# valeoai/NAF

Measured on AMD Instinct MI355X. Metric: upsampled Mpixels/sec (NAF forward), higher is better.
Workload: dtype bf16; 1 GPU; G1: 1x3x1024x1024 guidance, 1x768x64x64 features -> 1024x1024, window 7, per GPU; per_gpu_batch=1, global_batch=1, parallelism=batch-shard x1, scope=whole forward (conv stem + RoPE/pool + attention), weights=random-init NAF() defaults (dim 256, 4 heads), streams=2

## Files before the change

### naf_amd/csrc/stem_conv1x1.hip

```cpp
#include <type_traits>

#include "naf_common.h"

struct StemConv1Params {
    const bf16_t* x;
    bf16_t* y;
    const bf16_t* w;
    const float* bias;
    const float* gamma;
    const float* beta;
    const double* stats_in;
    double* stats_out;
    int32_t B, H, W;
    int32_t groups_per_image;
    int32_t groups_per_block;
    float eps;
    int64_t xs[3], ys[3];
    const void* img;
    const float* w0;
    const float* b0;
    int64_t ibs;
    int32_t is[4];
    bf16_t* kout;
    const float* tab_y;
    const float* tab_x;
    int64_t kst[3];
    int32_t cw;
    int32_t ncell;
    int32_t cells_per_block;
};

namespace {
constexpr int C1 = 128, WROW = C1 + 8, OROW1 = C1 + 8;
#ifndef NAF_C1X1_NW
#define NAF_C1X1_NW 4
#endif
#ifndef NAF_C1_ABL
#define NAF_C1_ABL 0
#endif
constexpr int NW1 = NAF_C1X1_NW;
typedef float f32x16_t __attribute__((ext_vector_type(16)));
constexpr float kLog2e = 1.4426950408889634f;
}

#ifdef NAF_C1_TIMING
__device__ unsigned long long g_c1_tim[4096 * 8];
#define C1_T(i) do { const unsigned long long now_ = __builtin_amdgcn_s_memtime(); tacc[i] += now_ - tlast; tlast = now_; } while (0)
#else
#define C1_T(i) do { } while (0)
#endif

template <bool IMG, typename T, bool DENSE, bool PLAIN = false, bool POOL = false>
__global__ __launch_bounds__(NW1 * 64, (NW1 <= 4 ? 2 : 1)) void stem_conv1x1_kernel(const StemConv1Params p) {
    static_assert(!(IMG && PLAIN), "the recomputed-conv0 input exists for the forward layer only");
    static_assert(!POOL || (DENSE && !IMG && !PLAIN), "key pooling: dense forward layer reading its input from memory");
#ifdef NAF_C1_TIMING
    unsigned long long tacc[8] = {0, 0, 0, 0, 0, 0, 0, 0}, tlast = __builtin_amdgcn_s_memtime();
#endif
    extern __shared__ __attribute__((aligned(16))) unsigned char smem[];
    bf16_t* wl = reinterpret_cast<bf16_t*>(smem);
    bf16_t* ot = wl + C1 * WROW;
    float* cvec = reinterpret_cast<float*>(ot + NW1 * 32 * OROW1);

    const int tid = threadIdx.x, lane = tid & 63;
    const int wave = __builtin_amdgcn_readfirstlane(tid >> 6);
    const int n32 = lane & 31, half = lane >> 5;
    const int b = blockIdx.y;

    const int gbase = POOL ? blockIdx.x * p.cells_per_block : blockIdx.x * p.groups_per_block;
    const int ngroups = POOL ? min(p.ncell, gbase + p.cells_per_block) : min(p.groups_per_image, gbase + p.groups_per_block);
    const int gstride = NW1;
    const int npx = p.H * p.W;
    bf16_t* otw = ot + wave * 32 * OROW1;

    const int chk = lane & 15, psub = lane >> 4;
    const bool xdense = DENSE || p.xs[1] == (int64_t)p.W * p.xs[2], ydense = DENSE || p.ys[1] == (int64_t)p.W * p.ys[2];
    const bf16_t* xbase = p.x + b * p.xs[0] + chk * 8;
    const uint32_t lane_x = (uint32_t)(psub * (int)p.xs[2] + chk * 8) * 2u, lane_y = (uint32_t)(psub * (int)p.ys[2] + chk * 8) * 2u;
    const int nfull = npx >> 5;
    auto pool_group_off = [&](int cell, int gi, const int64_t (&st)[3]) __attribute__((always_inline)) {
        const int cc = cell < ngroups ? cell : ngroups - 1;
        const int cy = cc / p.cw, cx = cc - cy * p.cw;
        return (int64_t)(cy * 16 + 2 * gi) * st[1] + (int64_t)cx * 16 * st[2];
    };
    auto load_group = [&](int g, u32x4_t (&raw)[8], int gi = 0) __attribute__((always_inline)) {
        if constexpr (POOL) {
            const char* xg = reinterpret_cast<const char*>(p.x + b * p.xs[0] + pool_group_off(g, gi, p.xs));
            uint32_t lx = lane_x;
            asm volatile("" : "+v"(lx));
#pragma unroll
            for (int it = 0; it < 8; ++it)
                raw[it] = *reinterpret_cast<const u32x4_t*>(xg + (uint32_t)(lx + (uint32_t)(((it >> 2) * (int)p.xs[1] + (it & 3) * 4 * (int)p.xs[2]) * 2)));
            return;
        }
        const int gc = g < ngroups ? g : ngroups - 1;
        if (DENSE || (xdense && gc < nfull)) {
            const char* xg = reinterpret_cast<const char*>(p.x + b * p.xs[0] + (int64_t)gc * 32 * p.xs[2]);
            uint32_t lx = lane_x;
            asm volatile("" : "+v"(lx));
#pragma unroll
            for (int it = 0; it < 8; ++it) raw[it] = *reinterpret_cast<const u32x4_t*>(xg + (uint32_t)(lx + (uint32_t)(it * 8 * (int)p.xs[2])));
            return;
        }
        if constexpr (!DENSE) {
#pragma unroll
        for (int it = 0; it < 8; ++it) {
            const int n = min(gc * 32 + it * 4 + psub, npx - 1);
            int64_t off;
            if (xdense) {
                off = (int64_t)n * p.xs[2];
            } else {
                const int yy = n / p.W, xx = n - yy * p.W;
                off = (int64_t)yy * p.xs[1] + (int64_t)xx * p.xs[2];
            }
            raw[it] = *reinterpret_cast<const u32x4_t*>(xbase + off);
        }
        }
    };
    constexpr int WCH = C1 * (C1 / 8), WIT = (WCH + NW1 * 64 - 1) / (NW1 * 64);
    u32x4_t wst[WIT];
#pragma unroll
    for (int i = 0; i < WIT; ++i) {
        const int ci = min(tid + i * NW1 * 64, WCH - 1);
        wst[i] = *reinterpret_cast<const u32x4_t*>(p.w + (ci >> 4) * C1 + (ci & 15) * 8);
    }
    u32x4_t raw[8];
    if constexpr (!IMG) load_group(gbase + wave, raw);
#pragma unroll
    for (int i = 0; i < WIT; ++i) {
        const int ci = tid + i * NW1 * 64;
        if (WCH % (NW1 * 64) == 0 || ci < WCH) *reinterpret_cast<u32x4_t*>(wl + (ci >> 4) * WROW + (ci & 15) * 8) = wst[i];
    }
    if (tid < C1) {
        const int c = tid, g = c >> 4;
        if constexpr (PLAIN) {
            cvec[c] = p.bias ? p.bias[c] : 0.f;
        } else {
            const double n = (double)p.H * (double)p.W * 16.0;
            double s1, s2;
            naf_gn_sums(p.stats_in, p.B, b, g, s1, s2);
            const double mean = s1 / n;
            double var = s2 / n - mean * mean;
            var = var > 0.0 ? var : 0.0;
            const float rstd = (float)(1.0 / sqrt(var + (double)p.eps));
            const float gmm = p.gamma[c];
            cvec[c] = p.bias[c];
            cvec[C1 + c] = gmm * rstd * kLog2e;
            cvec[2 * C1 + c] = (p.beta[c] - (float)mean * gmm * rstd) * kLog2e;
            if constexpr (IMG) cvec[3 * C1 + c] = p.b0[c];
        }
    }
    __syncthreads();

    float ga[8], gb[8];
#pragma unroll
    for (int e = 0; e < 8; ++e) {
        ga[e] = cvec[C1 + chk * 8 + e];
        gb[e] = cvec[2 * C1 + chk * 8 + e];
    }

    f32x2_t s1p[8], s2p[8];
#pragma unroll
    for (int g = 0; g < 8; ++g) s1p[g] = s2p[g] = f32x2_t{0.f, 0.f};

    float w0r[4][2];
    const T* ib = nullptr;
    if constexpr (IMG) {
        ib = reinterpret_cast<const T*>(p.img) + (int64_t)b * p.ibs;
#pragma unroll
        for (int m = 0; m < 4; ++m)
#pragma unroll
            for (int ks = 0; ks < 2; ++ks) {
                const int k = 2 * ks + half;
                w0r[m][ks] = (k < 3) ? p.w0[(32 * m + n32) * 3 + k] : 0.f;
            }
    }
    auto load_taps = [&](int g, float (&sv)[2]) __attribute__((always_inline)) {
        const int gc = g < ngroups ? g : ngroups - 1;
        const int n = min(gc * 32 + n32, npx - 1);
        const int yy = n / p.W, xx = n - yy * p.W;
        const int o = yy * p.is[2] + xx * p.is[3];
        sv[0] = (float)ib[o + half * p.is[1]];
        sv[1] = (float)ib[o + 2 * p.is[1]];
    };

    float sv[2] = {0.f, 0.f};
    int g = gbase + wave;
    int gi = 0;
    f32x4_t pacc[8];
    float ptab[16];
    bf16x8_t pax;
    const int pG = lane >> 4, pli = lane & 15;
    if constexpr (POOL) {
#pragma unroll
        for (int j = 0; j < 8; ++j) pacc[j] = f32x4_t{0.f, 0.f, 0.f, 0.f};
#pragma unroll
        for (int i = 0; i < 16; ++i) ptab[i] = 0.f;
#pragma unroll
        for (int i = 0; i < 8; ++i) pax[i] = (bf16_t)((8 * (pG & 1) + i == pli) ? 1.0f : 0.0f);
    }
    if constexpr (IMG) load_taps(g, sv);
    if constexpr (IMG) asm volatile("; conv1x1 first group landed" ::"v"(sv[0]), "v"(sv[1]));
    else asm volatile("; conv1x1 first group landed" ::"v"(raw[0]), "v"(raw[1]), "v"(raw[2]), "v"(raw[3]), "v"(raw[4]), "v"(raw[5]), "v"(raw[6]), "v"(raw[7]));
    C1_T(0);
    for (; g < ngroups; g += (POOL ? 0 : gstride)) {
        const int n0 = g * 32;
#ifdef NAF_C1_TIMING
        if constexpr (!IMG) {
            asm volatile("s_waitcnt vmcnt(8)" ::: "memory");
            C1_T(1);
        }
#endif
        const float* cv = cvec;

        f32x16_t acc[4];
#pragma unroll
        for (int m = 0; m < 4; ++m)
#pragma unroll
            for (int j = 0; j < 4; ++j) {
                const f32x4_t bj = *reinterpret_cast<const f32x4_t*>(cv + 32 * m + 8 * j + 4 * half);
#pragma unroll
                for (int i = 0; i < 4; ++i) acc[m][j * 4 + i] = bj[i];
            }
        if constexpr (IMG) {
#pragma unroll
            for (int mp = 0; mp < 2; ++mp) {
                f32x16_t a0[2];
#pragma unroll
                for (int q = 0; q < 2; ++q) {
#pragma unroll
                    for (int r = 0; r < 16; ++r) a0[q][r] = 0.f;
#pragma unroll
                    for (int ks = 0; ks < 2; ++ks) a0[q] = __builtin_amdgcn_mfma_f32_32x32x2f32(w0r[2 * mp + q][ks], sv[ks], a0[q], 0, 0, 0);
                }
#pragma unroll
                for (int q = 0; q < 2; ++q) {
                    const int m = 2 * mp + q;
#pragma unroll
                    for (int j = 0; j < 4; ++j) {
                        const int c0 = 32 * m + 8 * j + 4 * half;
                        const f32x4_t bj = *reinterpret_cast<const f32x4_t*>(cv + 3 * C1 + c0);
                        const f32x4_t gaj = *reinterpret_cast<const f32x4_t*>(cv + C1 + c0);
                        const f32x4_t gbj = *reinterpret_cast<const f32x4_t*>(cv + 2 * C1 + c0);
                        bf16x4_t o;
#pragma unroll
                        for (int e = 0; e < 2; ++e) {
                            const f32x2_t v = f32x2_t{a0[q][j * 4 + 2 * e], a0[q][j * 4 + 2 * e + 1]} + f32x2_t{bj[2 * e], bj[2 * e + 1]};
                            bf16x2_t xb;
                            xb[0] = (bf16_t)v[0];
                            xb[1] = (bf16_t)v[1];
                            const f32x2_t x = {(float)xb[0], (float)xb[1]};
                            const f32x2_t y = x * f32x2_t{gaj[2 * e], gaj[2 * e + 1]} + f32x2_t{gbj[2 * e], gbj[2 * e + 1]};
                            const f32x2_t u = f32x2_t{__builtin_amdgcn_exp2f(-y[0]), __builtin_amdgcn_exp2f(-y[1])} * kLog2e + kLog2e;
                            const f32x2_t r = y * f32x2_t{__builtin_amdgcn_rcpf(u[0]), __builtin_amdgcn_rcpf(u[1])};
                            o[2 * e] = (bf16_t)r[0];
                            o[2 * e + 1] = (bf16_t)r[1];
                        }
                        *reinterpret_cast<bf16x4_t*>(otw + n32 * OROW1 + c0) = o;
                    }
                }
            }
        } else {
#pragma unroll
        for (int it = 0; it < 8; ++it) {
            if constexpr (PLAIN || (NAF_C1_ABL & 1)) {
                *reinterpret_cast<u32x4_t*>(otw + (it * 4 + psub) * OROW1 + chk * 8) = raw[it];
                continue;
            }
            bf16x8_t o;
#pragma unroll
            for (int e = 0; e < 4; ++e) {
                const uint32_t w = raw[it][e];
                const f32x2_t x = {__uint_as_float(w << 16), __uint_as_float(w & 0xffff0000u)};
                const f32x2_t y = x * f32x2_t{ga[2 * e], ga[2 * e + 1]} + f32x2_t{gb[2 * e], gb[2 * e + 1]};
                const f32x2_t u = f32x2_t{__builtin_amdgcn_exp2f(-y[0]), __builtin_amdgcn_exp2f(-y[1])} * kLog2e + kLog2e;
                const f32x2_t r = y * f32x2_t{__builtin_amdgcn_rcpf(u[0]), __builtin_amdgcn_rcpf(u[1])};
                o[2 * e] = (bf16_t)r[0];
                o[2 * e + 1] = (bf16_t)r[1];
            }
            *reinterpret_cast<bf16x8_t*>(otw + (it * 4 + psub) * OROW1 + chk * 8) = o;
        }
        }
        C1_T(2);
        __builtin_amdgcn_sched_barrier(0);
        if constexpr (IMG) load_taps(g + gstride, sv);
        else if constexpr (POOL) {
            load_group(gi == 7 ? g + gstride : g, raw, (gi + 1) & 7);
            if (gi == 7) {
                const int cy = g / p.cw, cx = g - cy * p.cw;
                const float* ty = p.tab_y + (int64_t)(cy * 16 + 4 * pG) * 32 + pli;
                const float* tx = p.tab_x + (int64_t)(cx * 16 + 4 * pG) * 32 + pli;
#pragma unroll
                for (int i = 0; i < 4; ++i) {
                    ptab[i] = ty[i * 32];
                    ptab[4 + i] = ty[i * 32 + 16];
                    ptab[8 + i] = tx[i * 32];
                    ptab[12 + i] = tx[i * 32 + 16];
                }
            }
        }
        else if constexpr (!(NAF_C1_ABL & 16)) load_group(g + gstride, raw);
        __builtin_amdgcn_sched_barrier(0);
        {
            bf16x8_t bfr[2], war[2][4];
            auto frag = [&](int ks, int slot) __attribute__((always_inline)) {
                bfr[slot] = *reinterpret_cast<const bf16x8_t*>(otw + n32 * OROW1 + ks * 16 + half * 8);
#pragma unroll
                for (int m = 0; m < 4; ++m) war[slot][m] = *reinterpret_cast<const bf16x8_t*>(wl + (m * 32 + n32) * WROW + ks * 16 + half * 8);
            };
            frag(0, 0);
#pragma unroll
            for (int ks = 0; ks < 8; ++ks) {
                __builtin_amdgcn_sched_barrier(0);
                if (ks + 1 < 8) frag(ks + 1, (ks + 1) & 1);
                __builtin_amdgcn_sched_barrier(0);
#pragma unroll
                for (int m = 0; m < 4; ++m) {
                    if constexpr (!(NAF_C1_ABL & 2)) acc[m] = __builtin_amdgcn_mfma_f32_32x32x16_bf16(war[ks & 1][m], bfr[ks & 1], acc[m], 0, 0, 0);
                    else asm volatile("" ::"v"(war[ks & 1][m]), "v"(bfr[ks & 1]));
                }
            }
            __builtin_amdgcn_sched_barrier(0);
        }
#ifdef NAF_C1_TIMING
        asm volatile("" ::"v"(acc[0]), "v"(acc[1]), "v"(acc[2]), "v"(acc[3]));
        C1_T(3);
#endif
        const bool full = DENSE || g < nfull;
        auto epilogue = [&](auto fullc) __attribute__((always_inline)) {
            constexpr bool FULL = decltype(fullc)::value;
            const float vmask = (FULL || (n0 + n32) < npx) ? 1.0f : 0.0f;
#pragma unroll
            for (int m = 0; m < 4; ++m)
#pragma unroll
                for (int j = 0; j < 4; ++j) {
                    const f32x2_t v0 = f32x2_t{acc[m][j * 4], acc[m][j * 4 + 1]}, v1 = f32x2_t{acc[m][j * 4 + 2], acc[m][j * 4 + 3]};
                    bf16x4_t o;
                    o[0] = (bf16_t)v0[0]; o[1] = (bf16_t)v0[1]; o[2] = (bf16_t)v1[0]; o[3] = (bf16_t)v1[1];
                    const f32x2_t w0 = FULL ? v0 : v0 * vmask, w1 = FULL ? v1 : v1 * vmask;
                    if constexpr (!(NAF_C1_ABL & 4) && !POOL) {
                        s1p[m * 2 + (j >> 1)] += w0 + w1;
                        s2p[m * 2 + (j >> 1)] += w0 * w0 + w1 * w1;
                    }
                    *reinterpret_cast<bf16x4_t*>(otw + n32 * OROW1 + 32 * m + 8 * j + 4 * half) = o;
                }
            C1_T(4);
            bf16_t* yb = p.y + b * p.ys[0];
            if constexpr (POOL) {
                char* yg = reinterpret_cast<char*>(yb + pool_group_off(g, gi, p.ys));
                uint32_t ly = lane_y;
                asm volatile("" : "+v"(ly));
#pragma unroll
                for (int it = 0; it < 8; ++it) {
                    const u32x4_t v = *reinterpret_cast<const u32x4_t*>(otw + (it * 4 + psub) * OROW1 + chk * 8);
                    *reinterpret_cast<u32x4_t*>(yg + (uint32_t)(ly + (uint32_t)(((it >> 2) * (int)p.ys[1] + (it & 3) * 4 * (int)p.ys[2]) * 2))) = v;
                }
                return;
            }
            if (FULL && (DENSE || ydense)) {
                char* yg = reinterpret_cast<char*>(yb + (int64_t)g * 32 * p.ys[2]);
                uint32_t ly = lane_y;
                asm volatile("" : "+v"(ly));
#pragma unroll
                for (int it = 0; it < 8; ++it) {
                    const u32x4_t v = *reinterpret_cast<const u32x4_t*>(otw + (it * 4 + psub) * OROW1 + chk * 8);
                    if constexpr (!(NAF_C1_ABL & 8)) *reinterpret_cast<u32x4_t*>(yg + (int64_t)it * 8 * p.ys[2] + ly) = v;
                    else asm volatile("" ::"v"(v));
                }
                C1_T(5);
                return;
            }
            if constexpr (!(FULL && DENSE)) {
#pragma unroll
            for (int it = 0; it < 8; ++it) {
                const int pp = it * 4 + psub, ch = chk;
                const int n = n0 + pp;
                if (n < npx) {
                    int64_t off;
                    if (ydense) {
                        off = (int64_t)n * p.ys[2];
                    } else {
                        const int yy = n / p.W, xx = n - yy * p.W;
                        off = (int64_t)yy * p.ys[1] + (int64_t)xx * p.ys[2];
                    }
                    const u32x4_t v = *reinterpret_cast<const u32x4_t*>(otw + pp * OROW1 + ch * 8);
                    *reinterpret_cast<u32x4_t*>(yb + off + ch * 8) = v;
                }
            }
            }
        };
        if constexpr (DENSE) {
            epilogue(std::true_type{});
        } else {
            if (full) epilogue(std::true_type{});
            else epilogue(std::false_type{});
        }
        if constexpr (POOL) {
            bf16x8_t pay;
            {
                const bf16_t one = (bf16_t)(((2 * gi + (pG >> 1)) == pli) ? 1.0f : 0.0f);
#pragma unroll
                for (int i = 0; i < 8; ++i) pay[i] = one;
            }
            const bf16_t* tb = otw + (8 * pG + (pli >> 2)) * OROW1 + (pli & 3) * 4;
#pragma unroll
            for (int j = 0; j < 8; ++j) {
                const bf16x4_t lo = __builtin_amdgcn_ds_read_tr16_b64_v4bf16((NAF_LDS bf16x4_t*)(tb + 16 * j));
                const bf16x4_t hi = __builtin_amdgcn_ds_read_tr16_b64_v4bf16((NAF_LDS bf16x4_t*)(tb + 4 * OROW1 + 16 * j));
                const bf16x8_t bt = {lo[0], lo[1], lo[2], lo[3], hi[0], hi[1], hi[2], hi[3]};
                pacc[j] = __builtin_amdgcn_mfma_f32_16x16x32_bf16((j & 1) ? pax : pay, bt, pacc[j], 0, 0, 0);
            }
            if (gi == 7) {
                const int cy = g / p.cw, cx = g - cy * p.cw;
                bf16_t* kc = p.kout + b * p.kst[0] + (int64_t)cy * p.kst[1] + (int64_t)cx * p.kst[2];
#pragma unroll
                for (int hh = 0; hh < 2; ++hh) {
                    float o[4] = {0.f, 0.f, 0.f, 0.f};
#pragma unroll
                    for (int i = 0; i < 4; ++i) {
                        float r1, r2;
                        naf_rope_rotate(pacc[4 * hh][i], pacc[4 * hh + 2][i], ptab[i], ptab[4 + i], r1, r2);
                        o[0] += r1;
                        o[2] += r2;
                        naf_rope_rotate(pacc[4 * hh + 1][i], pacc[4 * hh + 3][i], ptab[8 + i], ptab[12 + i], r1, r2);
                        o[1] += r1;
                        o[3] += r2;
                    }
#pragma unroll
                    for (int q = 0; q < 4; ++q) {
                        o[q] += __shfl_xor(o[q], 16);
                        o[q] += __shfl_xor(o[q], 32);
                    }
                    const float v = pG == 0 ? o[0] : pG == 1 ? o[1] : pG == 2 ? o[2] : o[3];
                    kc[64 * hh + lane] = (bf16_t)(v * (1.0f / 256.0f));
                }
#pragma unroll
                for (int j = 0; j < 8; ++j) pacc[j] = f32x4_t{0.f, 0.f, 0.f, 0.f};
                gi = 0;
                g += gstride;
            } else {
                ++gi;
            }
        }
    }

    if constexpr (IMG) asm volatile("; conv1x1 loop drained" ::"v"(sv[0]), "v"(sv[1]));
    else asm volatile("; conv1x1 loop drained" ::"v"(raw[0]), "v"(raw[1]), "v"(raw[2]), "v"(raw[3]), "v"(raw[4]), "v"(raw[5]), "v"(raw[6]), "v"(raw[7]));
#ifdef NAF_C1_TIMING
    if (lane == 0 && blockIdx.x < 512)
        for (int i = 0; i < 8; ++i) g_c1_tim[(blockIdx.x * NW1 + wave) * 8 + i] = tacc[i];
#endif
    if (p.stats_out) {
        __syncthreads();
        float* red = reinterpret_cast<float*>(ot);
#pragma unroll
        for (int gq = 0; gq < 8; ++gq) {
            float a = s1p[gq][0] + s1p[gq][1], q = s2p[gq][0] + s2p[gq][1];
#pragma unroll
            for (int o = 32; o > 0; o >>= 1) {
                a += __shfl_xor(a, o);
                q += __shfl_xor(q, o);
            }
            if (lane == 0) {
                red[wave * 16 + gq] = a;
                red[wave * 16 + 8 + gq] = q;
            }
        }
        __syncthreads();
        if (tid < 16) {
            float a = 0.f;
#pragma unroll
            for (int wv = 0; wv < NW1; ++wv) a += red[wv * 16 + tid];
            atomicAdd(&naf_gn_slot(p.stats_out, p.B, b, blockIdx.x)[(tid & 7) * 2 + (tid >> 3)], (double)a);
        }
    }
}

int naf_stem_conv1x1_keys_ok(const naf_stem_conv_args* a, const naf_key_pool_args* kp) {
    return a->ksize == 1 && a->first == nullptr && a->stats_in != nullptr && a->stats_out == nullptr && (a->channels == 0 || a->channels == 128) &&
           a->H == 16 * kp->h && a->W == 16 * kp->w && a->x_stride[1] == (int64_t)a->W * a->x_stride[2] &&
           a->y_stride[1] == (int64_t)a->W * a->y_stride[2] && a->x_stride[1] * 2 < 0x7fffffffLL && a->y_stride[1] * 2 < 0x7fffffffLL;
}

int naf_launch_stem_conv1x1(const naf_stem_conv_args* a, hipStream_t s, const naf_key_pool_args* kp) {
    StemConv1Params p;
    p.x = static_cast<const bf16_t*>(a->x);
    p.y = static_cast<bf16_t*>(a->y);
    p.w = static_cast<const bf16_t*>(a->w_packed);
    p.bias = a->bias; p.gamma = a->gn_weight; p.beta = a->gn_bias;
    p.stats_in = a->stats_in; p.stats_out = a->stats_out;
    p.B = a->B; p.H = a->H; p.W = a->W; p.eps = a->eps;
    for (int i = 0; i < 3; ++i) { p.xs[i] = a->x_stride[i]; p.ys[i] = a->y_stride[i]; }
    p.groups_per_image = (int)(((int64_t)a->H * a->W + 31) / 32);
    const size_t lds = (size_t)(C1 * WROW + NW1 * 32 * OROW1) * 2 + 4 * C1 * sizeof(float);
    const int64_t slots = (int64_t)naf_cu_count() * (NW1 <= 4 ? 2 : 1) * NW1;
    const int64_t total = (int64_t)p.groups_per_image * a->B;
    const int64_t gpw = (total + slots - 1) / slots;
    static const int gpw_knob = [] { const char* e = naf_knob("NAF_C1X1_GPW"); return e ? atoi(e) : 0; }();
    const int64_t gpw_eff = gpw_knob > 0 ? gpw_knob : gpw;
    p.groups_per_block = (int32_t)(gpw_eff * NW1);
    int64_t nbx = (p.groups_per_image + p.groups_per_block - 1) / p.groups_per_block;
    if (nbx < 1) nbx = 1;
    if (a->B > 65535) {
        naf_set_error("naf_stem_conv_fwd: batch %d out of range", a->B);
        return NAF_ERR_INVALID;
    }
    p.img = nullptr; p.w0 = nullptr; p.b0 = nullptr; p.ibs = 0;
    for (int i = 0; i < 4; ++i) p.is[i] = 0;
    p.kout = nullptr; p.tab_y = p.tab_x = nullptr; p.cw = p.ncell = p.cells_per_block = 0;
    for (int i = 0; i < 3; ++i) p.kst[i] = 0;
    if (kp != nullptr) {
        if (!naf_stem_conv1x1_keys_ok(a, kp)) {
            naf_set_error("naf_stem_conv_keys_fwd: the 1x1 kernel needs 16 x 16 pixel cells, dense rows, stats_out == NULL and first == NULL");
            return NAF_ERR_UNSUPPORTED;
        }
        p.kout = static_cast<bf16_t*>(kp->k_lr); p.tab_y = kp->tab_y; p.tab_x = kp->tab_x;
        for (int i = 0; i < 3; ++i) p.kst[i] = kp->k_stride[i];
        p.cw = kp->w; p.ncell = kp->h * kp->w;
        const int64_t cpw = ((int64_t)p.ncell * a->B + slots - 1) / slots;
        p.cells_per_block = (int32_t)(cpw * NW1);
        nbx = (p.ncell + p.cells_per_block - 1) / p.cells_per_block;
    }
    int variant = 0;
    if (a->first != nullptr) {
        const naf_stem_conv0_args* f = a->first;
        const int64_t span = 2 * llabs(f->image_stride[1]) + (int64_t)(a->H - 1) * llabs(f->image_stride[2]) +
                             (int64_t)(a->W - 1) * llabs(f->image_stride[3]);
        if (span >= 0x7fffffffLL) {
            naf_set_error("naf_stem_conv_fwd: first: image too large for 32-bit tap offsets (span %lld elements)", (long long)span);
            return NAF_ERR_UNSUPPORTED;
        }
        p.img = f->image; p.w0 = f->weight; p.b0 = f->bias; p.ibs = f->image_stride[0];
        for (int i = 0; i < 4; ++i) p.is[i] = (int32_t)f->image_stride[i];
        variant = f->image_dtype == NAF_BF16 ? 2 : 1;
    }
    const dim3 grid((uint32_t)nbx, (uint32_t)a->B), blk(NW1 * 64);
    if (kp != nullptr) {
        auto kern = stem_conv1x1_kernel<false, float, true, false, true>;
        if (hipFuncSetAttribute(reinterpret_cast<const void*>(kern), hipFuncAttributeMaxDynamicSharedMemorySize, (int)lds) != hipSuccess) {
            naf_set_error("naf_stem_conv_keys_fwd: cannot reserve %zu bytes of LDS", (size_t)lds);
            return NAF_ERR_LAUNCH;
        }
        hipLaunchKernelGGL(kern, grid, blk, lds, s, p);
        return naf_check_launch("stem_conv1x1_kernel<keys>");
    }
#define NAF_LAUNCH_1X1(KERN)                                                                                              \
    do {                                                                                                                  \
        if (hipFuncSetAttribute(reinterpret_cast<const void*>(KERN), hipFuncAttributeMaxDynamicSharedMemorySize, (int)lds) != hipSuccess) { \
            naf_set_error("naf_stem_conv_fwd: cannot reserve %zu bytes of LDS", (size_t)lds);                             \
            return NAF_ERR_LAUNCH;                                                                                        \
        }                                                                                                                 \
        hipLaunchKernelGGL(KERN, grid, blk, lds, s, p);                                                                   \
    } while (0)
    const bool dense = (a->x_stride[1] == (int64_t)a->W * a->x_stride[2] || a->first != nullptr) &&
                       a->y_stride[1] == (int64_t)a->W * a->y_stride[2] && (((int64_t)a->H * a->W) % 32 == 0);
    if (a->stats_in == nullptr) {
        if (dense) NAF_LAUNCH_1X1((stem_conv1x1_kernel<false, float, true, true>));
        else NAF_LAUNCH_1X1((stem_conv1x1_kernel<false, float, false, true>));
    } else if (dense) {
        if (variant == 0) NAF_LAUNCH_1X1((stem_conv1x1_kernel<false, float, true>));
        else if (variant == 1) NAF_LAUNCH_1X1((stem_conv1x1_kernel<true, float, true>));
        else NAF_LAUNCH_1X1((stem_conv1x1_kernel<true, bf16_t, true>));
    } else {
        if (variant == 0) NAF_LAUNCH_1X1((stem_conv1x1_kernel<false, float, false>));
        else if (variant == 1) NAF_LAUNCH_1X1((stem_conv1x1_kernel<true, float, false>));
        else NAF_LAUNCH_1X1((stem_conv1x1_kernel<true, bf16_t, false>));
    }
#undef NAF_LAUNCH_1X1
    return naf_check_launch("stem_conv1x1_kernel");
}
```

Before: 566.5 Mpix/s.

## Fold first 3-channel conv into main 1x1 path via 16x16x4 MFMA

Replaces the separate IMG-path epilogue, which used two 32x32x2 MFMAs per 32-channel block plus its own GroupNorm/SiLU loop, with a 16x16x4 MFMA that computes the 3-tap conv and bias together. Its bf16 results feed the existing raw[] normalization/SiLU loop, so both paths share one code path. The bias row moves out of the LDS cvec table and into registers, and image taps are loaded with a lane mapping matched to the new MFMA layout. A dense fast path for tap addressing is added, and dense mode now also requires W divisible by 32 when the first layer is fused.

```diff
diff --git a/naf_amd/csrc/stem_conv1x1.hip b/naf_amd/csrc/stem_conv1x1.hip
--- a/naf_amd/csrc/stem_conv1x1.hip
+++ b/naf_amd/csrc/stem_conv1x1.hip
@@ -147,7 +147,6 @@
             cvec[c] = p.bias[c];
             cvec[C1 + c] = gmm * rstd * kLog2e;
             cvec[2 * C1 + c] = (p.beta[c] - (float)mean * gmm * rstd) * kLog2e;
-            if constexpr (IMG) cvec[3 * C1 + c] = p.b0[c];
         }
     }
     __syncthreads();
@@ -163,25 +162,29 @@
 #pragma unroll
     for (int g = 0; g < 8; ++g) s1p[g] = s2p[g] = f32x2_t{0.f, 0.f};
 
-    float w0r[4][2];
+    float wb0[8];
     const T* ib = nullptr;
     if constexpr (IMG) {
-        ib = reinterpret_cast<const T*>(p.img) + (int64_t)b * p.ibs;
-#pragma unroll
-        for (int m = 0; m < 4; ++m)
-#pragma unroll
-            for (int ks = 0; ks < 2; ++ks) {
-                const int k = 2 * ks + half;
-                w0r[m][ks] = (k < 3) ? p.w0[(32 * m + n32) * 3 + k] : 0.f;
-            }
-    }
+        ib = reinterpret_cast<const T*>(p.img) + (int64_t)b * p.ibs + min(psub, 2) * p.is[1];
+#pragma unroll
+        for (int e = 0; e < 8; ++e) wb0[e] = psub < 3 ? p.w0[(chk * 8 + e) * 3 + psub] : p.b0[chk * 8 + e];
+    }
+    const int tpx = 4 * (chk & 3) + (chk >> 2);
     auto load_taps = [&](int g, float (&sv)[2]) __attribute__((always_inline)) {
         const int gc = g < ngroups ? g : ngroups - 1;
-        const int n = min(gc * 32 + n32, npx - 1);
-        const int yy = n / p.W, xx = n - yy * p.W;
-        const int o = yy * p.is[2] + xx * p.is[3];
-        sv[0] = (float)ib[o + half * p.is[1]];
-        sv[1] = (float)ib[o + 2 * p.is[1]];
+#pragma unroll
+        for (int h = 0; h < 2; ++h) {
+            int o;
+            if constexpr (DENSE) {
+                const int yy = (gc * 32) / p.W, x0 = gc * 32 - yy * p.W;
+                o = yy * p.is[2] + x0 * p.is[3] + (16 * h + tpx) * p.is[3];
+            } else {
+                const int n = min(gc * 32 + 16 * h + tpx, npx - 1);
+                const int yy = n / p.W, xx = n - yy * p.W;
+                o = yy * p.is[2] + xx * p.is[3];
+            }
+            sv[h] = (float)ib[o];
+        }
     };
 
     float sv[2] = {0.f, 0.f};
@@ -222,47 +225,28 @@
 #pragma unroll
                 for (int i = 0; i < 4; ++i) acc[m][j * 4 + i] = bj[i];
             }
+#ifdef NAF_C1_TIMING
         if constexpr (IMG) {
-#pragma unroll
-            for (int mp = 0; mp < 2; ++mp) {
-                f32x16_t a0[2];
-#pragma unroll
-                for (int q = 0; q < 2; ++q) {
-#pragma unroll
-                    for (int r = 0; r < 16; ++r) a0[q][r] = 0.f;
-#pragma unroll
-                    for (int ks = 0; ks < 2; ++ks) a0[q] = __builtin_amdgcn_mfma_f32_32x32x2f32(w0r[2 * mp + q][ks], sv[ks], a0[q], 0, 0, 0);
-                }
-#pragma unroll
-                for (int q = 0; q < 2; ++q) {
-                    const int m = 2 * mp + q;
-#pragma unroll
-                    for (int j = 0; j < 4; ++j) {
-                        const int c0 = 32 * m + 8 * j + 4 * half;
-                        const f32x4_t bj = *reinterpret_cast<const f32x4_t*>(cv + 3 * C1 + c0);
-                        const f32x4_t gaj = *reinterpret_cast<const f32x4_t*>(cv + C1 + c0);
-                        const f32x4_t gbj = *reinterpret_cast<const f32x4_t*>(cv + 2 * C1 + c0);
-                        bf16x4_t o;
-#pragma unroll
-                        for (int e = 0; e < 2; ++e) {
-                            const f32x2_t v = f32x2_t{a0[q][j * 4 + 2 * e], a0[q][j * 4 + 2 * e + 1]} + f32x2_t{bj[2 * e], bj[2 * e + 1]};
-                            bf16x2_t xb;
-                            xb[0] = (bf16_t)v[0];
-                            xb[1] = (bf16_t)v[1];
-                            const f32x2_t x = {(float)xb[0], (float)xb[1]};
-                            const f32x2_t y = x * f32x2_t{gaj[2 * e], gaj[2 * e + 1]} + f32x2_t{gbj[2 * e], gbj[2 * e + 1]};
-                            const f32x2_t u = f32x2_t{__builtin_amdgcn_exp2f(-y[0]), __builtin_amdgcn_exp2f(-y[1])} * kLog2e + kLog2e;
-                            const f32x2_t r = y * f32x2_t{__builtin_amdgcn_rcpf(u[0]), __builtin_amdgcn_rcpf(u[1])};
-                            o[2 * e] = (bf16_t)r[0];
-                            o[2 * e + 1] = (bf16_t)r[1];
-                        }
-                        *reinterpret_cast<bf16x4_t*>(otw + n32 * OROW1 + c0) = o;
-                    }
-                }
-            }
-        } else {
+            asm volatile("" ::"v"(sv[0]), "v"(sv[1]));
+            C1_T(1);
+        }
+#endif
+        f32x4_t c0r[8];
 #pragma unroll
         for (int it = 0; it < 8; ++it) {
+            if constexpr (IMG) {
+                if ((it & 3) == 0) {
+                    const float x = sv[it >> 2], ak = psub < 3 ? x : __builtin_fmaf(0.f, x, 1.0f);
+#pragma unroll
+                    for (int e = 0; e < 8; ++e) c0r[e] = __builtin_amdgcn_mfma_f32_16x16x4f32(ak, wb0[e], f32x4_t{0.f, 0.f, 0.f, 0.f}, 0, 0, 0);
+                }
+#pragma unroll
+                for (int e = 0; e < 4; ++e) {
+                    uint32_t w = __builtin_bit_cast(uint32_t, __builtin_convertvector(f32x2_t{c0r[2 * e][it & 3], c0r[2 * e + 1][it & 3]}, bf16x2_t));
+                    asm("" : "+v"(w));
+                    raw[it][e] = w;
+                }
+            }
             if constexpr (PLAIN || (NAF_C1_ABL & 1)) {
                 *reinterpret_cast<u32x4_t*>(otw + (it * 4 + psub) * OROW1 + chk * 8) = raw[it];
                 continue;
@@ -279,7 +263,6 @@
                 o[2 * e + 1] = (bf16_t)r[1];
             }
             *reinterpret_cast<bf16x8_t*>(otw + (it * 4 + psub) * OROW1 + chk * 8) = o;
-        }
         }
         C1_T(2);
         __builtin_amdgcn_sched_barrier(0);
@@ -492,7 +475,7 @@
     p.B = a->B; p.H = a->H; p.W = a->W; p.eps = a->eps;
     for (int i = 0; i < 3; ++i) { p.xs[i] = a->x_stride[i]; p.ys[i] = a->y_stride[i]; }
     p.groups_per_image = (int)(((int64_t)a->H * a->W + 31) / 32);
-    const size_t lds = (size_t)(C1 * WROW + NW1 * 32 * OROW1) * 2 + 4 * C1 * sizeof(float);
+    const size_t lds = (size_t)(C1 * WROW + NW1 * 32 * OROW1) * 2 + 3 * C1 * sizeof(float);
     const int64_t slots = (int64_t)naf_cu_count() * (NW1 <= 4 ? 2 : 1) * NW1;
     const int64_t total = (int64_t)p.groups_per_image * a->B;
     const int64_t gpw = (total + slots - 1) / slots;
@@ -553,7 +536,8 @@
         hipLaunchKernelGGL(KERN, grid, blk, lds, s, p);                                                                   \
     } while (0)
     const bool dense = (a->x_stride[1] == (int64_t)a->W * a->x_stride[2] || a->first != nullptr) &&
-                       a->y_stride[1] == (int64_t)a->W * a->y_stride[2] && (((int64_t)a->H * a->W) % 32 == 0);
+                       a->y_stride[1] == (int64_t)a->W * a->y_stride[2] && (((int64_t)a->H * a->W) % 32 == 0) &&
+                       (a->first == nullptr || a->W % 32 == 0);
     if (a->stats_in == nullptr) {
         if (dense) NAF_LAUNCH_1X1((stem_conv1x1_kernel<false, float, true, true>));
         else NAF_LAUNCH_1X1((stem_conv1x1_kernel<false, float, false, true>));
```

Result: no change. 568.8 Mpix/s (median of 6 runs) (+0.4%).
